# w111liang222/lidar-slam-detection

Hardware: AMD Instinct MI355X
Metric: registered points/sec (120k-pt scan vs 1e7-pt map, full iterate-to-converge) (higher is better)
Workload: dtype f32 per-point geometry / f64 transforms and reductions

## Files before the change

### lidar-slam-detection_amd/csrc/batch.hip

```cpp
#include <sched.h>
#include <stdlib.h>

#include <chrono>
#include <deque>
#include <vector>

#include "eskf.h"
#include "lio_common.h"

using namespace lio;

int engine_resume_update(lio_engine* e, const double* x_now26, const double* x_prop26, const double* P_prop, int i, int converge, int t);
void engine_count_passes(lio_engine* e, int* n_pass, int* n_knn);
int engine_joint_register_device(lio_engine* e, const void* d_raw, uint32_t n_raw, double lidar_beg_time, double state26[26], double cov[529]);
struct lio_comm;
extern "C" int lio_comm_world(const lio_comm*);
extern "C" {
int engine_seq_prepare(lio_engine* e, uint32_t n_raw, double lidar_beg_time, int* ekf_inited);
void engine_seq_params(lio_engine* e, double* laser_cov, int* maximum_iter, int* degenerate_detect_en, float* leaf_surf, float* leaf_map, int* static_map,
                       double* travel, double last_pos_lid[3]);
int engine_seq_finish(lio_engine* e, const double x26[26], const double P529[529], int n_ds, int n_pass, int n_knn, int n_eff, int degenerate, int inserted,
                      uint32_t n_add, uint32_t map_err, uint32_t bound);
int engine_seq_resume(lio_engine* e, const double* x_now26, const double* x_prop26, const double* P_prop, int i, int converge, int t);
int engine_seq_has_lru(lio_engine* e);
int engine_fastlio_front(lio_engine* e, const void** d_raw, uint32_t* n_raw, double* beg, double state26[26], double cov529[529]);
void engine_fastlio_back(lio_engine* e);
}

namespace {

struct Group {
    hipStream_t stream = nullptr;
    std::vector<lio_engine*> eng;
    std::vector<lio_engine*> sub_eng;
    double* d_local32 = nullptr;
    double* d_gathered = nullptr;
    char* d_ds_send = nullptr;
    char* d_ds_all = nullptr;
    int ds_world = 0;
    MapRef* d_rowmaps = nullptr;
    std::vector<MapRef> rowmap_rows;
    char* d_block = nullptr;
    char* h_block = nullptr;
    size_t block_bytes = 0;
    SlotDesc* d_desc = nullptr;
    SlotDesc* h_desc = nullptr;
    EskfDev* d_ctrl = nullptr;
    EskfDev* h_ctrl = nullptr;
    hipGraphExec_t exec[5] = {nullptr, nullptr, nullptr, nullptr, nullptr};
    const void* graph_table = nullptr;
    int graph_stencil = 0;
    lio_batch_result* h_res = nullptr;
    lio_batch_result* h_res_dev = nullptr;
    std::vector<int> job_of_slot;
    float4* d_rawbuf = nullptr;
    MapRef* d_maps = nullptr;
    MapRef* h_maps = nullptr;
    SeqDev* d_seq = nullptr;
    SeqDev* h_seq = nullptr;
    std::vector<int> seq_path;
    int any_lru = 0;
    int n_active = 0;
    int launched_passes = 4;
    uint32_t seq = 0;
    uint32_t max_n_raw = 0;
    BatchTimer* bt = nullptr;
};

}

struct lio_batch {
    lio_map* map = nullptr;
    int device = 0;
    int n_slots = 0;
    uint32_t max_raw = 0, max_ds = 0;
    int pred_passes = 4;
    bool broken = false;
    int use_graph = 1;
    int count_touched = 0;
    std::vector<lio_map*> maps;
    lio_comm* comm = nullptr;
    int world = 1;
    int rank = 0;
    int split_ds = 1;
    uint32_t ds_cap = 0;
    uint32_t ds_seen_max = 0;
    bool ds_cap_full = false;
    uint64_t n_ds_cut = 0;
    int (*gather_hook)(void*, const double*, double*, uint32_t, void*) = nullptr;
    void* gather_ctx = nullptr;
    bool joint = false;
    bool sequences = false;
    std::vector<lio_scan_job> fl_jobs;
    std::vector<double> fl_state, fl_cov;
    std::vector<Group> groups;
    double t_submit = 0, t_wait = 0, t_collect = 0;
    uint64_t n_rounds = 0;
};

static void fill_mapref(MapRef& r, const lio_map* m);

namespace {

const MapRef* joint_rowmaps(lio_batch* b, Group& g) {
    const int M = (int)b->maps.size(), B = b->n_slots;
    if (M < 2) return nullptr;
    for (int m = 1; m < M; m++)
        if (b->maps[m]->stencil_id != b->maps[0]->stencil_id || b->maps[m]->stencil.n != b->maps[0]->stencil.n) return nullptr;
    std::vector<MapRef> now((size_t)M);
    for (int m = 0; m < M; m++) {
        memset(&now[m], 0, sizeof(MapRef));
        fill_mapref(now[m], b->maps[m]);
    }
    bool fresh = g.d_rowmaps != nullptr && (int)g.rowmap_rows.size() == M;
    for (int m = 0; m < M && fresh; m++) fresh = memcmp(&g.rowmap_rows[m], &now[m], sizeof(MapRef)) == 0;
    if (fresh) return g.d_rowmaps;
    std::vector<MapRef> rows((size_t)M * B);
    for (int m = 0; m < M; m++)
        for (int s = 0; s < B; s++) rows[(size_t)m * B + s] = now[m];
    if (!g.d_rowmaps && hipMalloc(reinterpret_cast<void**>(&g.d_rowmaps), sizeof(MapRef) * rows.size()) != hipSuccess) { g.d_rowmaps = nullptr; return nullptr; }
    if (hipMemcpyAsync(g.d_rowmaps, rows.data(), sizeof(MapRef) * rows.size(), hipMemcpyHostToDevice, g.stream) != hipSuccess) return nullptr;
    if (hipStreamSynchronize(g.stream) != hipSuccess) return nullptr;
    g.rowmap_rows = now;
    return g.d_rowmaps;
}

void fill_desc(SlotDesc& d, lio_scan* sc, EskfDev* d_ctrl, lio_batch_result* d_res) {
    d.max_ds = sc->max_ds;
    d.partial_blocks = sc->partial_blocks;
    d.sd = sc->dev;
    d.keys_a = sc->keys_a; d.keys_b = sc->keys_b; d.vals_a = sc->vals_a; d.vals_b = sc->vals_b;
    d.hist = sc->hist; d.blockcnt = sc->blockcnt; d.hpos = sc->hpos; d.longlist = sc->longlist; d.tie_list = sc->tie_list;
    d.sorted = sc->sorted; d.ds_body = sc->ds_body; d.ds_world = sc->ds_world; d.nn_pts = sc->nn_pts; d.normvec = sc->normvec;
    d.nn_cnt = sc->nn_cnt; d.selected = sc->selected; d.partial = sc->partial;
    d.host_nds = sc->host_nds_dev;
    d.ctrl = d_ctrl;
    d.result = d_res;
}

void fill_ctrl(EskfDev& c, const double* x26, const double* P529, double R, int max_iter, int degenerate_detect_en, int joint = 0) {
    c.joint = joint;
    memcpy(c.x, x26, sizeof(double) * 26);
    memcpy(c.P, P529, sizeof(double) * 529);
    for (int k = 0; k < kEkN; k++) c.limit[k] = 0.001;
    c.R = R;
    c.maximum_iter = max_iter;
    c.degenerate_detect_en = degenerate_detect_en;
    c.is_degenerate = 0;
    ek_begin(c);
}

void group_free(Group& g) {
    for (lio_engine* e : g.eng) lio_engine_destroy(e);
    for (lio_engine* e : g.sub_eng) lio_engine_destroy(e);
    if (g.d_local32) hipFree(g.d_local32);
    if (g.d_gathered) hipFree(g.d_gathered);
    if (g.d_ds_send) hipFree(g.d_ds_send);
    if (g.d_ds_all) hipFree(g.d_ds_all);
    if (g.d_rowmaps) hipFree(g.d_rowmaps);
    for (int k = 0; k < 5; k++)
        if (g.exec[k]) hipGraphExecDestroy(g.exec[k]);
    if (g.d_block) hipFree(g.d_block);
    if (g.d_rawbuf) hipFree(g.d_rawbuf);
    if (g.h_block) hipHostFree(g.h_block);
    if (g.d_seq) hipFree(g.d_seq);
    if (g.h_seq) hipHostFree(g.h_seq);
    if (g.h_res) hipHostFree(g.h_res);
    if (g.stream) hipStreamDestroy(g.stream);
    if (g.bt) {
        if (g.bt->created)
            for (int c = 0; c < BatchTimer::kClasses; c++)
                for (int i = 0; i < BatchTimer::kPool; i++) { hipEventDestroy(g.bt->ev[c][i][0]); hipEventDestroy(g.bt->ev[c][i][1]); }
        delete g.bt;
    }
}

const float4* stage_host_raw(lio_batch* b, Group& g, int slot, const lio_scan_job& job, int* rc) {
    *rc = LIO_OK;
    if (!g.d_rawbuf) {
        if (hipMalloc(reinterpret_cast<void**>(&g.d_rawbuf), sizeof(float4) * (size_t)b->max_raw * (size_t)b->n_slots) != hipSuccess) {
            set_error("lio_batch: no memory for the raw ring of LIO_JOB_HOST_RAW jobs (%d x %u points)", b->n_slots, b->max_raw);
            *rc = LIO_E_DEVICE;
            return nullptr;
        }
    }
    float4* dst = g.d_rawbuf + (size_t)slot * b->max_raw;
    if (hipMemcpyAsync(dst, job.d_raw, sizeof(float4) * (size_t)job.n_raw, hipMemcpyHostToDevice, g.stream) != hipSuccess) {
        set_error("lio_batch: copy of a LIO_JOB_HOST_RAW cloud failed: %s", hipGetErrorString(hipGetLastError()));
        *rc = LIO_E_DEVICE;
        return nullptr;
    }
    return dst;
}

int submit(lio_batch* b, Group& g, lio_scan_job* jobs, int first, int n, int passes) {
    const int B = b->n_slots;
    g.seq++;
    g.n_active = 0;
    g.max_n_raw = 0;
    g.launched_passes = passes;
    for (int s = 0; s < B; s++) {
        SlotDesc& d = g.h_desc[s];
        d.active = 0;
        g.job_of_slot[s] = -1;
        if (s >= n) continue;
        lio_scan_job& job = jobs[first + s];
        g.job_of_slot[s] = first + s;
        job.rc = LIO_E_INVALID;
        job.n_ds = job.n_pass = job.n_knn_pass = 0;
        if (job.flags & ~LIO_JOB_FLAGS_KNOWN) { set_error("lio_scan_job.flags = 0x%x: unknown bits (a job array that was not zero-initialised?)", job.flags); continue; }
        if (job.flags & LIO_JOB_IDLE) { job.rc = 0; g.job_of_slot[s] = -1; continue; }
        if (!job.state_in || !job.cov_in || (!job.d_raw && job.n_raw)) continue;
        if (job.n_raw > b->max_raw) { set_error("scan of %u points exceeds max_raw %u", job.n_raw, b->max_raw); job.rc = LIO_E_CAPACITY; continue; }
        if (job.n_raw == 0) { job.rc = 2; continue; }
        d.raw = static_cast<const float4*>(job.d_raw);
        if (job.flags & LIO_JOB_HOST_RAW) {
            int src = LIO_OK;
            d.raw = stage_host_raw(b, g, s, job, &src);
            if (src != LIO_OK) { job.rc = src; continue; }
        }
        d.n_raw = job.n_raw;
        d.nblocks = (job.n_raw + 2047u) / 2048u;
        d.active = 1;
        d.seq = g.seq;
        d.min_ds = 5;
        d.reset_cache = (job.flags & LIO_JOB_KEEP_CACHE) ? 0u : 1u;
        fill_ctrl(g.h_ctrl[s], job.state_in, job.cov_in, 0.001 , 4, 1, b->joint ? 1 : 0);
        g.h_res[s].seq = g.seq - 1;
        g.n_active++;
        if (job.n_raw > g.max_n_raw) g.max_n_raw = job.n_raw;
    }
    const int M = (int)b->maps.size();
    for (int m = 1; m < M; m++)
        for (int s = 0; s < B; s++) {
            SlotDesc& d = g.h_desc[(size_t)m * B + s];
            const SlotDesc& p = g.h_desc[s];
            d.raw = p.raw; d.n_raw = p.n_raw; d.nblocks = p.nblocks; d.active = p.active; d.seq = p.seq; d.min_ds = p.min_ds; d.reset_cache = p.reset_cache;
        }
    if (g.n_active == 0) return LIO_OK;
    const bool timed = g.bt && g.bt->on;
    const MapRef* rowmaps = b->joint ? joint_rowmaps(b, g) : nullptr;
    auto enqueue = [&](BatchTimer* bt) -> int {
        LIO_HIP_TRY(hipMemcpyAsync(g.d_block, g.h_block, g.block_bytes, hipMemcpyHostToDevice, g.stream));
        const uint32_t ds_bound = b->max_raw < b->max_ds ? b->max_raw : b->max_ds;
        int rc = LIO_OK;
        if (b->joint && b->world > 1 && b->split_ds) {
            const int per = (B + b->world - 1) / b->world;
            const int s0 = std::min(B, b->rank * per), s1 = std::min(B, s0 + per);
            if (g.ds_world != b->world) {
                if (g.d_ds_send) hipFree(g.d_ds_send);
                if (g.d_ds_all) hipFree(g.d_ds_all);
                g.d_ds_send = g.d_ds_all = nullptr;
                g.ds_world = 0;
                const size_t chunk = (size_t)per * ds_exchange_slot_bytes(ds_bound);
                LIO_HIP_TRY(hipMalloc(reinterpret_cast<void**>(&g.d_ds_send), chunk));
                LIO_HIP_TRY(hipMalloc(reinterpret_cast<void**>(&g.d_ds_all), chunk * (size_t)b->world));
                g.ds_world = b->world;
            }
            if (bt) bt->begin(0);
            if (s1 > s0) rc = vg_downsample_batch(g.stream, g.d_desc + s0, s1 - s0, b->max_raw, b->max_ds, 0.5f, passes);
            if (bt) bt->end(0);
            if (rc != LIO_OK) return rc;
            if (b->ds_cap == 0) {
                const char* k = getenv("LIO_JOINT_DS_CAP");
                const uint32_t want = k ? (uint32_t)strtoul(k, nullptr, 10) : ((ds_bound / 4u + 1023u) & ~1023u);
                b->ds_cap = std::min(ds_bound, std::max(k ? 1u : 4096u, want));
            }
            const uint32_t cap = b->ds_cap_full ? ds_bound : b->ds_cap;
            rc = p2plane_batch_exchange_ds(b->comm, b->world, b->gather_hook, b->gather_ctx, g.stream, g.d_desc, B, per, s0, s1, cap, g.d_ds_send, g.d_ds_all);
            if (rc == LIO_OK && s0 > 0) rc = scan_begin_rows(g.stream, g.d_desc, s0);
            if (rc == LIO_OK && s1 < B) rc = scan_begin_rows(g.stream, g.d_desc + s1, B - s1);
            if (rc != LIO_OK) return rc;
        } else {
            if (bt) bt->begin(0);
            rc = vg_downsample_batch(g.stream, g.d_desc, B, b->max_raw, b->max_ds, 0.5f, passes);
            if (bt) bt->end(0);
            if (rc != LIO_OK) return rc;
        }
        if (b->joint) {
            rc = p2plane_batch_share(g.stream, g.d_desc, B, M, ds_bound);
            if (rc == LIO_OK) rc = scan_begin_rows(g.stream, g.d_desc + B, B * (M - 1));
            if (rc != LIO_OK) return rc;
            return p2plane_batch_update_joint(b->maps.data(), M, b->comm, b->world, b->gather_hook, b->gather_ctx, g.stream, g.d_desc, B, ds_bound, 5, g.d_local32, g.d_gathered, bt,
                                              rowmaps);
        }
        return p2plane_batch_update(b->map, g.stream, g.d_desc, B, ds_bound, 5, bt, bt ? b->count_touched : 0);
    };
    if (!b->use_graph || timed || b->joint) return enqueue(timed ? g.bt : nullptr);
    if (g.graph_table != b->map->table || g.graph_stencil != b->map->stencil.n) {
        for (int k = 0; k < 5; k++)
            if (g.exec[k]) { hipGraphExecDestroy(g.exec[k]); g.exec[k] = nullptr; }
        g.graph_table = b->map->table;
        g.graph_stencil = b->map->stencil.n;
    }
    if (!g.exec[passes]) {
        hipGraph_t graph = nullptr;
        LIO_HIP_TRY(hipStreamBeginCapture(g.stream, hipStreamCaptureModeThreadLocal));
        const int rc = enqueue(nullptr);
        const hipError_t e2 = hipStreamEndCapture(g.stream, &graph);
        if (rc != LIO_OK) { if (graph) hipGraphDestroy(graph); return rc; }
        LIO_HIP_TRY(e2);
        LIO_HIP_TRY(hipGraphInstantiate(&g.exec[passes], graph, nullptr, nullptr, 0));
        hipGraphDestroy(graph);
    }
    LIO_HIP_TRY(hipGraphLaunch(g.exec[passes], g.stream));
    return LIO_OK;
}

int wait_group(Group& g, int B) {
    for (int s = 0; s < B; s++) {
        if (!g.h_desc[s].active) continue;
        volatile uint32_t* seq = &g.h_res[s].seq;
        for (uint64_t spin = 0; *seq != g.seq; spin++) {
            __builtin_ia32_pause();
            if (spin > 2000 && (spin & 31) == 0) sched_yield();
            if (spin > 40000000ull) {
                LIO_HIP_TRY(hipStreamSynchronize(g.stream));
                if (*seq != g.seq) { set_error("batch slot %d did not report (seq %u, expected %u)", s, *seq, g.seq); return LIO_E_DEVICE; }
                break;
            }
        }
    }
    __atomic_thread_fence(__ATOMIC_ACQUIRE);
    return LIO_OK;
}

}


extern "C" {

static lio_batch* batch_create_impl(lio_map** maps, int n_maps, lio_comm* comm, int n_slots, int n_groups, uint32_t max_raw, uint32_t max_ds) {
    lio_map* map = n_maps > 0 && maps ? maps[0] : nullptr;
    if (!map || n_maps > 64 || n_slots < 1 || n_slots > 256 || n_groups < 1 || n_groups > 8 || max_raw == 0 || max_ds == 0) { set_error("lio_batch_create: bad argument"); return nullptr; }
    for (int m = 1; m < n_maps; m++)
        if (!maps[m] || maps[m]->device != map->device) { set_error("lio_batch_create_joint: the sub-maps of a batch live on one device"); return nullptr; }
    if (hipSetDevice(map->device) != hipSuccess) { set_error("lio_batch_create: no HIP device %d", map->device); return nullptr; }
    lio_batch* b = new lio_batch();
    b->map = map;
    b->device = map->device;
    b->n_slots = n_slots;
    b->max_raw = max_raw;
    b->max_ds = max_ds;
    b->maps.assign(maps, maps + n_maps);
    b->comm = comm;
    b->world = comm ? lio_comm_world(comm) : 1;
    b->rank = comm ? lio_comm_rank(comm) : 0;
    { const char* k = getenv("LIO_JOINT_SPLIT_DS"); b->split_ds = (k && k[0] == '0') ? 0 : 1; }
    b->joint = n_maps > 1 || comm != nullptr;
    b->groups.resize(n_groups);
    { const char* k = getenv("LIO_BATCH_GRAPH"); b->use_graph = (k && k[0] == '0') ? 0 : 1; }
    bool ok = true;
    const int M = n_maps;
    for (Group& g : b->groups) ok = ok && hipStreamCreateWithFlags(&g.stream, hipStreamNonBlocking) == hipSuccess;
    for (Group& g : b->groups) {
        g.job_of_slot.assign(n_slots, -1);
        const size_t desc_bytes = sizeof(SlotDesc) * (size_t)n_slots * (size_t)M;
        g.block_bytes = desc_bytes + sizeof(EskfDev) * (size_t)n_slots;
        ok = ok && hipMalloc(reinterpret_cast<void**>(&g.d_block), g.block_bytes) == hipSuccess;
        ok = ok && hipHostMalloc(reinterpret_cast<void**>(&g.h_block), g.block_bytes, hipHostMallocDefault) == hipSuccess;
        if (ok) {
            g.d_desc = reinterpret_cast<SlotDesc*>(g.d_block);
            g.h_desc = reinterpret_cast<SlotDesc*>(g.h_block);
            g.d_ctrl = reinterpret_cast<EskfDev*>(g.d_block + desc_bytes);
            g.h_ctrl = reinterpret_cast<EskfDev*>(g.h_block + desc_bytes);
        }
        ok = ok && hipHostMalloc(reinterpret_cast<void**>(&g.h_res), sizeof(lio_batch_result) * n_slots, hipHostMallocMapped) == hipSuccess;
        ok = ok && hipHostGetDevicePointer(reinterpret_cast<void**>(&g.h_res_dev), g.h_res, 0) == hipSuccess;
        if (b->joint) {
            ok = ok && hipMalloc(reinterpret_cast<void**>(&g.d_local32), sizeof(double) * 32 * n_slots) == hipSuccess;
            ok = ok && hipMalloc(reinterpret_cast<void**>(&g.d_gathered), sizeof(double) * 32 * n_slots * (size_t)b->world) == hipSuccess;
        }
        if (!ok) break;
        memset(g.h_block, 0, g.block_bytes);
        memset(g.h_res, 0, sizeof(lio_batch_result) * n_slots);
        ok = hipMemset(g.d_block, 0, g.block_bytes) == hipSuccess;
        for (int s = 0; s < n_slots && ok; s++) {
            lio_engine* e = lio_engine_create_shared(map, max_raw, max_ds);
            if (!e) { ok = false; break; }
            lio_engine_set_flags(e, 1, 0, 0.0, -10.0);
            g.eng.push_back(e);
            fill_desc(g.h_desc[s], lio_engine_scan(e), &g.d_ctrl[s], &g.h_res_dev[s]);
        }
        for (int m = 1; m < M && ok; m++)
            for (int s = 0; s < n_slots && ok; s++) {
                lio_engine* e = lio_engine_create_shared(maps[m], max_raw, max_ds);
                if (!e) { ok = false; break; }
                lio_engine_set_flags(e, 1, 0, 0.0, -10.0);
                g.sub_eng.push_back(e);
                fill_desc(g.h_desc[(size_t)m * n_slots + s], lio_engine_scan(e), &g.d_ctrl[s], nullptr);
            }
        for (int s = 0; s < n_slots && ok && b->joint; s++) {
            std::vector<lio_engine*> others;
            for (int m = 1; m < M; m++) others.push_back(g.sub_eng[(size_t)(m - 1) * n_slots + s]);
            ok = lio_engine_set_joint(g.eng[s], others.empty() ? nullptr : others.data(), (int)others.size(), comm) == LIO_OK;
        }
    }
    if (!ok) {
        set_error("lio_batch_create: device setup failed: %s", hipGetErrorString(hipGetLastError()));
        lio_batch_destroy(b);
        return nullptr;
    }
    {
        const char* q = getenv("GPU_MAX_HW_QUEUES");
        if (n_groups > 1 && (!q || atoi(q) < 8))
            set_warning("lio_batch_create: GPU_MAX_HW_QUEUES=%s -- with fewer than 8 hardware queues the %d rounds in flight mostly serialise (~20 %% slower); "
                        "export GPU_MAX_HW_QUEUES=8 before the process's first HIP call", q ? q : "(unset: 4)", n_groups);
    }
    return b;
}

lio_batch* lio_batch_create(lio_map* map, int n_slots, int n_groups, uint32_t max_raw, uint32_t max_ds) {
    return batch_create_impl(&map, map ? 1 : 0, nullptr, n_slots, n_groups, max_raw, max_ds);
}

lio_batch* lio_batch_create_joint(lio_map** sub_maps, int n_sub_maps, lio_comm* comm, int n_slots, int n_groups, uint32_t max_raw, uint32_t max_ds) {
    return batch_create_impl(sub_maps, n_sub_maps, comm, n_slots, n_groups, max_raw, max_ds);
}

int lio_batch_set_gather_hook(lio_batch* b, lio_gather_fn fn, void* ctx, int rank, int world) {
    if (!b || !fn || world < 1 || rank < 0 || rank >= world) return LIO_E_INVALID;
    if (!b->joint || b->comm) { set_error("lio_batch_set_gather_hook: for a batch made by lio_batch_create_joint without a communicator"); return LIO_E_STATE; }
    hipSetDevice(b->map->device);
    for (auto& g : b->groups) {
        LIO_HIP_TRY(hipStreamSynchronize(g.stream));
        if (g.d_gathered) hipFree(g.d_gathered);
        g.d_gathered = nullptr;
        LIO_HIP_TRY(hipMalloc(reinterpret_cast<void**>(&g.d_gathered), sizeof(double) * 32 * b->n_slots * (size_t)world));
    }
    b->gather_hook = fn;
    b->gather_ctx = ctx;
    b->world = world;
    b->rank = rank;
    return LIO_OK;
}

int lio_batch_exchange_stats(lio_batch* b, uint32_t* chunk_points, uint64_t* jobs_rerun, uint64_t* bytes_per_rank_and_round) {
    if (!b) return LIO_E_INVALID;
    const bool on = b->joint && b->world > 1 && b->split_ds;
    if (chunk_points) *chunk_points = on ? b->ds_cap : 0u;
    if (jobs_rerun) *jobs_rerun = b->n_ds_cut;
    if (bytes_per_rank_and_round) {
        const int per = (b->n_slots + b->world - 1) / b->world;
        *bytes_per_rank_and_round = on && b->ds_cap ? (uint64_t)per * ds_exchange_slot_bytes(b->ds_cap) : 0u;
    }
    return LIO_OK;
}

void lio_batch_destroy(lio_batch* b) {
    if (!b) return;
    hipSetDevice(b->device);
    if (getenv("LIO_BATCH_PROFILE") && b->n_rounds)
        fprintf(stderr, "lio_batch: %llu rounds of %d slots; host per round: submit %.1f us, wait %.1f us, collect %.1f us\n", (unsigned long long)b->n_rounds,
                b->n_slots, 1e6 * b->t_submit / b->n_rounds, 1e6 * b->t_wait / b->n_rounds, 1e6 * b->t_collect / b->n_rounds);
    for (Group& g : b->groups) {
        if (g.stream) hipStreamSynchronize(g.stream);
        group_free(g);
    }
    delete b;
}

int lio_batch_enable_kernel_timing(lio_batch* b, int on) {
    if (!b) return LIO_E_INVALID;
    hipSetDevice(b->device);
    for (Group& g : b->groups) {
        if (!g.bt) { g.bt = new BatchTimer(); g.bt->stream = g.stream; }
        if (on && !g.bt->created) {
            for (int c = 0; c < BatchTimer::kClasses; c++)
                for (int i = 0; i < BatchTimer::kPool; i++) {
                    LIO_HIP_TRY(hipEventCreate(&g.bt->ev[c][i][0]));
                    LIO_HIP_TRY(hipEventCreate(&g.bt->ev[c][i][1]));
                }
            g.bt->created = true;
        }
        g.bt->on = on != 0;
    }
    b->count_touched = (on & 2) ? 1 : 0;
    if (b->count_touched && b->map) { const int rc = map_enable_touch_bits(b->map); if (rc != LIO_OK) return rc; }
    return LIO_OK;
}

int lio_batch_kernel_times(lio_batch* b, lio_batch_times* out, int reset) {
    if (!b || !out) return LIO_E_INVALID;
    memset(out, 0, sizeof(*out));
    for (Group& g : b->groups) {
        if (!g.bt) continue;
        out->downsample_us += g.bt->us[0]; out->knn_us += g.bt->us[1]; out->linearize_us += g.bt->us[2]; out->step_us += g.bt->us[3];
        out->downsample_launches += g.bt->launches[0]; out->knn_launches += g.bt->launches[1]; out->linearize_launches += g.bt->launches[2];
        out->step_launches += g.bt->launches[3];
        out->insert_us += g.bt->us[4];
        out->insert_launches += g.bt->launches[4];
        if (reset)
            for (int c = 0; c < BatchTimer::kClasses; c++) { g.bt->us[c] = 0; g.bt->launches[c] = 0; }
    }
    return LIO_OK;
}

lio_engine* lio_batch_engine(lio_batch* b, int group, int slot) {
    if (!b || group < 0 || group >= (int)b->groups.size() || slot < 0 || slot >= b->n_slots) return nullptr;
    return b->groups[group].eng[slot];
}

int lio_batch_process(lio_batch* b, lio_scan_job* jobs, int n_jobs) {
    if (!b || (!jobs && n_jobs) || n_jobs < 0) return LIO_E_INVALID;
    if (b->sequences) { set_error("lio_batch_process: a sequence batch is driven by lio_batch_sequences_step"); return LIO_E_STATE; }
    hipSetDevice(b->device);
    const int B = b->n_slots;
    int next = 0, first_err = 0;
    std::deque<int> inflight;
    std::vector<int> retry;
    auto note = [&](int rc) { if (rc < 0 && !first_err) first_err = rc; };
    auto collect = [&](Group& g) {
        int need_max = 1;
        for (int s = 0; s < B; s++) {
            const int j = g.job_of_slot[s];
            if (j < 0) continue;
            if (!g.h_desc[s].active) { note(jobs[j].rc); continue; }
            lio_scan_job& job = jobs[j];
            const lio_batch_result& r = g.h_res[s];
            if (r.radix_passes > need_max) need_max = r.radix_passes;
            if (r.radix_passes > g.launched_passes) { retry.push_back(j); continue; }
            lio_engine* e = g.eng[s];
            lio_scan* sc = lio_engine_scan(e);
            sc->have_ds = r.n_ds;
            sc->n_raw = g.h_desc[s].n_raw;
            job.n_ds = r.n_ds;
            job.n_pass = r.n_pass;
            job.n_knn_pass = r.n_knn_pass;
            if (r.err & 4) {
                hipMemsetAsync(&sc->dev->err, 0, 4, g.stream);
                b->n_ds_cut++;
                retry.push_back(j);
                continue;
            }
            if (r.err & 1) {
                set_error("downsampled scan exceeds max_ds %u", b->max_ds);
                hipMemsetAsync(&sc->dev->err, 0, 4, g.stream);
                job.rc = LIO_E_CAPACITY;
                note(job.rc);
                continue;
            }
            if ((uint32_t)r.n_ds > b->ds_seen_max) b->ds_seen_max = (uint32_t)r.n_ds;
            if (r.status == EK_SKIPPED) { job.rc = 2; continue; }
            if (r.status == EK_NEEDS_HOST && b->joint && b->gather_hook) {
                set_error("lio_batch (gather hook mode): a scan needs the host-driven joint path, which only exists over a lio_comm");
                job.rc = LIO_E_STATE;
                note(job.rc);
                continue;
            }
            if (r.status == EK_NEEDS_HOST && b->joint) {
                if (!(job.flags & LIO_JOB_KEEP_CACHE)) {
                    scan_forget_cache(sc);
                    for (int m = 1; m < (int)b->maps.size(); m++) scan_forget_cache(lio_engine_scan(g.sub_eng[(size_t)(m - 1) * B + s]));
                }
                double st26[26], cov[529];
                memcpy(st26, job.state_in, sizeof(st26));
                memcpy(cov, job.cov_in, sizeof(cov));
                const void* d_cloud = (job.flags & LIO_JOB_HOST_RAW) ? static_cast<const void*>(g.d_rawbuf + (size_t)s * b->max_raw) : job.d_raw;
                const int rc = engine_joint_register_device(e, d_cloud, job.n_raw, job.lidar_beg_time, st26, cov);
                if (rc < 0) { job.rc = rc; note(rc); continue; }
                engine_count_passes(e, &job.n_pass, &job.n_knn_pass);
                if (job.state_out) memcpy(job.state_out, st26, sizeof(st26));
                job.rc = rc;
                continue;
            }
            if (r.status == EK_NEEDS_HOST) {
                const int rc = engine_resume_update(e, r.state, job.state_in, job.cov_in, r.loop_i, r.loop_converge, r.loop_t);
                if (rc != LIO_OK) { job.rc = rc; note(rc); continue; }
                int np = 0, nk = 0;
                engine_count_passes(e, &np, &nk);
                job.n_pass += np;
                job.n_knn_pass += nk;
                if (job.state_out) lio_engine_get_state(e, job.state_out);
                job.rc = 3;
                continue;
            }
            if (job.state_out) memcpy(job.state_out, r.state, sizeof(double) * 26);
            job.rc = 3;
        }
        if (need_max > 4) need_max = 4;
        b->pred_passes = need_max;
        if (b->joint && b->world > 1 && b->split_ds && b->ds_seen_max && !getenv("LIO_JOINT_DS_CAP")) {
            const uint32_t ds_bound = b->max_raw < b->max_ds ? b->max_raw : b->max_ds;
            const uint32_t want = (b->ds_seen_max + b->ds_seen_max / 4u + 1023u) & ~1023u;
            b->ds_cap = std::min(ds_bound, std::max(4096u, want));
        }
    };
    using clk = std::chrono::steady_clock;
    auto secs = [](clk::time_point a, clk::time_point c) { return std::chrono::duration<double>(c - a).count(); };
    auto bail = [&](int rc) {
        for (auto& gg : b->groups) hipStreamSynchronize(gg.stream);
        inflight.clear();
        return rc;
    };
    for (size_t gi = 0; gi < b->groups.size() && next < n_jobs; gi++) {
        const int n = n_jobs - next < B ? n_jobs - next : B;
        const auto t0 = clk::now();
        const int rc = submit(b, b->groups[gi], jobs, next, n, b->pred_passes);
        b->t_submit += secs(t0, clk::now());
        b->n_rounds++;
        if (rc != LIO_OK) return bail(rc);
        next += n;
        inflight.push_back((int)gi);
    }
    while (!inflight.empty()) {
        const int gi = inflight.front();
        inflight.pop_front();
        Group& g = b->groups[gi];
        const auto t0 = clk::now();
        if (g.n_active) {
            const int rc = wait_group(g, B);
            if (rc != LIO_OK) return bail(rc);
        }
        if (g.bt && g.bt->on) { hipStreamSynchronize(g.stream); g.bt->resolve(); }
        const auto t1 = clk::now();
        collect(g);
        const auto t2 = clk::now();
        b->t_wait += secs(t0, t1);
        b->t_collect += secs(t1, t2);
        if (next < n_jobs) {
            const int n = n_jobs - next < B ? n_jobs - next : B;
            const int rc = submit(b, g, jobs, next, n, b->pred_passes);
            b->t_submit += secs(t2, clk::now());
            b->n_rounds++;
            if (rc != LIO_OK) return bail(rc);
            next += n;
            inflight.push_back(gi);
        }
    }
    const std::vector<int> todo = retry;
    retry.clear();
    b->ds_cap_full = true;
    for (const int j : todo) {
        Group& g = b->groups[0];
        int rc = submit(b, g, jobs, j, 1, 4);
        if (rc == LIO_OK && g.n_active) rc = wait_group(g, B);
        if (rc != LIO_OK) { b->ds_cap_full = false; return bail(rc); }
        collect(g);
    }
    b->ds_cap_full = false;
    for (const int j : retry) { jobs[j].rc = LIO_E_DEVICE; note(LIO_E_DEVICE); }
    return first_err;
}

static void fill_mapref(MapRef& r, const lio_map* m) {
    r.table = m->table; r.cap = m->cap; r.pending = m->pending; r.created = m->created; r.pool = m->pool; r.pool_seq = m->pool_seq; r.tie_mode = m->tie_mode; r.md = m->dev;
    r.slot_of_point = m->slot_of_point; r.stage = m->stage; r.pool_cap = m->pool_cap;
    r.touch = m->touch; r.prev_touch = m->prev_touch; r.lru_log = m->lru_log; r.log_mask = m->lru_log_cap ? m->lru_log_cap - 1 : 0;
    r.free_items = m->free_items; r.free_in = m->free_in; r.free_cap = m->free_cap;
    r.first_touch = m->first_touch; r.lru_g = m->lru_g; r.lru_rec = m->lru_rec;
    r.lru_capacity = (uint32_t)m->lru_capacity; r.lru_max_distance = m->lru_max_distance;
    r.mask = m->table_mask; r.inv_res = m->inv_res; r.res = m->res; r.key_mode = m->key_mode; r.max_voxels = (uint32_t)m->max_voxels;
    r.stencil_id = m->stencil_id;
}

lio_batch* lio_batch_create_sequences(int device, float resolution, int stencil, uint64_t max_points, uint64_t max_voxels, int n_slots, int n_groups,
                                      uint32_t max_raw, uint32_t max_ds) {
    if (n_slots < 1 || n_slots > 256 || n_groups < 1 || n_groups > 8 || max_raw == 0 || max_ds == 0 || max_points == 0 || max_voxels == 0) {
        set_error("lio_batch_create_sequences: bad argument");
        return nullptr;
    }
    const uint32_t ds_bound = max_raw < max_ds ? max_raw : max_ds;
    if (ds_bound > max_points || ds_bound > (1u << 20)) { set_error("lio_batch_create_sequences: a scan's %u downsampled points exceed the maps' insert scratch", ds_bound); return nullptr; }
    if (hipSetDevice(device) != hipSuccess) { set_error("lio_batch_create_sequences: no HIP device %d", device); return nullptr; }
    lio_batch* b = new lio_batch();
    b->device = device;
    b->n_slots = n_slots;
    b->max_raw = max_raw;
    b->max_ds = max_ds;
    b->sequences = true;
    { const char* k = getenv("LIO_BATCH_GRAPH"); b->use_graph = (k && k[0] == '0') ? 0 : 1; }
    b->groups.resize(n_groups);
    bool ok = true;
    for (Group& g : b->groups) ok = ok && hipStreamCreateWithFlags(&g.stream, hipStreamNonBlocking) == hipSuccess;
    for (Group& g : b->groups) {
        g.job_of_slot.assign(n_slots, -1);
        g.seq_path.assign(n_slots, 0);
        const size_t desc_bytes = sizeof(SlotDesc) * (size_t)n_slots, ctrl_bytes = sizeof(EskfDev) * (size_t)n_slots;
        g.block_bytes = desc_bytes + ctrl_bytes + sizeof(MapRef) * (size_t)n_slots;
        ok = ok && hipMalloc(reinterpret_cast<void**>(&g.d_block), g.block_bytes) == hipSuccess;
        ok = ok && hipHostMalloc(reinterpret_cast<void**>(&g.h_block), g.block_bytes, hipHostMallocDefault) == hipSuccess;
        ok = ok && hipMalloc(reinterpret_cast<void**>(&g.d_seq), sizeof(SeqDev) * (size_t)n_slots) == hipSuccess;
        ok = ok && hipHostMalloc(reinterpret_cast<void**>(&g.h_seq), sizeof(SeqDev) * (size_t)n_slots, hipHostMallocDefault) == hipSuccess;
        ok = ok && hipHostMalloc(reinterpret_cast<void**>(&g.h_res), sizeof(lio_batch_result) * n_slots, hipHostMallocMapped) == hipSuccess;
        ok = ok && hipHostGetDevicePointer(reinterpret_cast<void**>(&g.h_res_dev), g.h_res, 0) == hipSuccess;
        if (!ok) break;
        g.d_desc = reinterpret_cast<SlotDesc*>(g.d_block);
        g.h_desc = reinterpret_cast<SlotDesc*>(g.h_block);
        g.d_ctrl = reinterpret_cast<EskfDev*>(g.d_block + desc_bytes);
        g.h_ctrl = reinterpret_cast<EskfDev*>(g.h_block + desc_bytes);
        g.d_maps = reinterpret_cast<MapRef*>(g.d_block + desc_bytes + ctrl_bytes);
        g.h_maps = reinterpret_cast<MapRef*>(g.h_block + desc_bytes + ctrl_bytes);
        memset(g.h_block, 0, g.block_bytes);
        memset(g.h_res, 0, sizeof(lio_batch_result) * n_slots);
        memset(g.h_seq, 0, sizeof(SeqDev) * (size_t)n_slots);
        ok = hipMemset(g.d_block, 0, g.block_bytes) == hipSuccess && hipMemset(g.d_seq, 0, sizeof(SeqDev) * (size_t)n_slots) == hipSuccess;
        for (int s = 0; s < n_slots && ok; s++) {
            lio_engine* e = lio_engine_create(device, resolution, stencil, max_points, max_voxels, max_raw, max_ds);
            if (!e) { ok = false; break; }
            lio_engine_set_device_loop(e, 1);
            g.eng.push_back(e);
            fill_desc(g.h_desc[s], lio_engine_scan(e), &g.d_ctrl[s], &g.h_res_dev[s]);
        }
    }
    if (!ok) {
        set_error("lio_batch_create_sequences: device setup failed: %s", hipGetErrorString(hipGetLastError()));
        lio_batch_destroy(b);
        return nullptr;
    }
    b->map = lio_engine_map(b->groups[0].eng[0]);
    return b;
}

int lio_batch_sequences_step(lio_batch* b, lio_scan_job* jobs, int n_jobs, double* cov_out) {
    if (!b || !jobs) return LIO_E_INVALID;
    if (!b->sequences) { set_error("lio_batch_sequences_step: for a batch made by lio_batch_create_sequences"); return LIO_E_STATE; }
    if (b->broken) { set_error("lio_batch_sequences_step: an earlier step failed after part of it had run on the device; the sessions' maps hold that sweep, their engines do not -- destroy the batch"); return LIO_E_STATE; }
    const int B = b->n_slots, G = (int)b->groups.size();
    if (n_jobs != B * G) { set_error("lio_batch_sequences_step: %d jobs for %d sessions (job j is the next scan of session j; LIO_JOB_IDLE marks a session without one)", n_jobs, B * G); return LIO_E_INVALID; }
    hipSetDevice(b->device);
    int first_err = 0;
    auto note = [&](int rc) { if (rc < 0 && !first_err) first_err = rc; };
    const uint32_t ds_bound = b->max_raw < b->max_ds ? b->max_raw : b->max_ds;
    const int passes = b->pred_passes;
    for (int gi = 0; gi < G; gi++) {
        Group& g = b->groups[gi];
        g.seq++;
        g.n_active = 0;
        g.max_n_raw = 0;
        g.launched_passes = passes;
        g.any_lru = 0;
        StencilArgs stencils[4];
        int stencil_ids[4], n_st = 0;
        for (int s = 0; s < B; s++) {
            SlotDesc& d = g.h_desc[s];
            d.active = 0;
            g.job_of_slot[s] = gi * B + s;
            g.seq_path[s] = -1000;
            lio_scan_job& job = jobs[gi * B + s];
            job.n_ds = job.n_pass = job.n_knn_pass = 0;
            job.rc = LIO_E_INVALID;
            if (job.flags & ~LIO_JOB_FLAGS_KNOWN) { set_error("lio_scan_job.flags = 0x%x: unknown bits (a job array that was not zero-initialised?)", job.flags); note(job.rc); continue; }
            if (job.flags & LIO_JOB_IDLE) { job.rc = 0; g.job_of_slot[s] = -1; continue; }
            if (!job.state_in || !job.cov_in || (!job.d_raw && job.n_raw)) { note(job.rc); continue; }
            if (job.flags & LIO_JOB_HOST_RAW) { set_error("lio_batch_sequences_step: LIO_JOB_HOST_RAW is a static-batch flag (a session's sweeps arrive through lio_fastlio_pcl_stage / _commit)"); note(job.rc); continue; }
            if (job.n_raw > b->max_raw) { set_error("scan of %u points exceeds max_raw %u", job.n_raw, b->max_raw); job.rc = LIO_E_CAPACITY; note(job.rc); continue; }
            lio_engine* e = g.eng[s];
            int ekf_inited = 0;
            const int path = engine_seq_prepare(e, job.n_raw, job.lidar_beg_time, &ekf_inited);
            g.seq_path[s] = path;
            if (path < 0) { job.rc = path; note(path); continue; }
            if (path == 0 || path == 2) { job.rc = path; if (job.state_out) memcpy(job.state_out, job.state_in, sizeof(double) * 26); if (cov_out) memcpy(cov_out + (size_t)(gi * B + s) * 529, job.cov_in, sizeof(double) * 529); continue; }
            if (path == 10) {
                lio_engine_set_state(e, job.state_in);
                lio_engine_set_cov(e, job.cov_in);
                const int rc = lio_engine_process_scan_device(e, job.d_raw, job.n_raw, job.lidar_beg_time);
                job.rc = rc;
                note(rc);
                if (rc >= 0) {
                    lio_timings tm;
                    lio_engine_timings(e, &tm);
                    job.n_ds = tm.n_ds; job.n_pass = tm.n_pass; job.n_knn_pass = tm.n_knn_pass;
                    if (job.state_out) lio_engine_get_state(e, job.state_out);
                    if (cov_out) lio_engine_get_cov(e, cov_out + (size_t)(gi * B + s) * 529);
                }
                continue;
            }
            lio_map* m = lio_engine_map(e);
            double laser_cov = 0.001, travel = 0, last_pos_lid[3];
            int maximum_iter = 4, deg_en = 1, static_map = 0;
            float leaf_surf = 0.5f, leaf_map = 0.5f;
            engine_seq_params(e, &laser_cov, &maximum_iter, &deg_en, &leaf_surf, &leaf_map, &static_map, &travel, last_pos_lid);
            if (leaf_surf != 0.5f || maximum_iter != 4) { set_error("sequence batch: the round is built for filter_size_surf 0.5 and NUM_MAX_ITERATIONS 4"); job.rc = LIO_E_STATE; note(job.rc); g.seq_path[s] = LIO_E_STATE; continue; }
            if (m->lru_capacity && m->tomb_bound > m->table_cap / 4) {
                const int rc = map_rebuild(m, g.stream);
                if (rc != LIO_OK) { job.rc = rc; note(rc); g.seq_path[s] = rc; continue; }
            }
            d.raw = static_cast<const float4*>(job.d_raw);
            d.n_raw = job.n_raw;
            d.nblocks = (job.n_raw + 2047u) / 2048u;
            d.active = 1;
            d.seq = g.seq;
            d.min_ds = 5;
            d.reset_cache = 0;
            fill_ctrl(g.h_ctrl[s], job.state_in, job.cov_in, laser_cov, maximum_iter, deg_en, 0);
            MapRef& r = g.h_maps[s];
            fill_mapref(r, m);
            r.stamp_base = (unsigned long long)(m->n_batches + 1) << kStampIdxBits;
            r.do_insert = static_map ? 0u : 1u;
            r.ekf_inited = (uint32_t)ekf_inited;
            r.map_leaf = leaf_map;
            r.travel_prev = travel;
            for (int i = 0; i < 3; i++) r.last_pos_lid[i] = last_pos_lid[i];
            if (m->lru_capacity) g.any_lru = 1;
            int k = 0;
            while (k < n_st && stencil_ids[k] != m->stencil_id) k++;
            if (k == n_st && n_st < 4) { stencils[n_st] = m->stencil; stencil_ids[n_st] = m->stencil_id; n_st++; }
            else if (k == n_st) { set_error("sequence batch: more than four different stencils in one round"); job.rc = LIO_E_STATE; note(job.rc); d.active = 0; g.seq_path[s] = LIO_E_STATE; continue; }
            g.h_res[s].seq = g.seq - 1;
            g.n_active++;
            if (job.n_raw > g.max_n_raw) g.max_n_raw = job.n_raw;
        }
        if (g.n_active == 0) continue;
        const bool timed = g.bt && g.bt->on;
        auto enqueue = [&](BatchTimer* bt) -> int {
            LIO_HIP_TRY(hipMemcpyAsync(g.d_block, g.h_block, g.block_bytes, hipMemcpyHostToDevice, g.stream));
            if (bt) bt->begin(0);
            int rc = vg_downsample_batch(g.stream, g.d_desc, B, b->max_raw, b->max_ds, 0.5f, passes);
            if (bt) bt->end(0);
            if (rc == LIO_OK) rc = p2plane_seq_update(g.stream, g.d_maps, g.d_desc, B, ds_bound, 5, stencils, stencil_ids, n_st, bt);
            if (bt) bt->begin(4);
            if (rc == LIO_OK) rc = p2plane_seq_insert(g.stream, g.d_maps, g.d_desc, g.d_seq, B, ds_bound, g.any_lru);
            if (bt) bt->end(4);
            if (rc != LIO_OK) return rc;
            LIO_HIP_TRY(hipMemcpyAsync(g.h_seq, g.d_seq, sizeof(SeqDev) * (size_t)B, hipMemcpyDeviceToHost, g.stream));
            return LIO_OK;
        };
        int rc = LIO_OK;
        if (!b->use_graph || timed) {
            rc = enqueue(timed ? g.bt : nullptr);
        } else {
            int sig = g.any_lru ? 1 : 0;
            for (int k = 0; k < n_st; k++) sig = sig * 131 + stencil_ids[k] + 1;
            if (g.graph_stencil != sig) {
                for (int k = 0; k < 5; k++)
                    if (g.exec[k]) { hipGraphExecDestroy(g.exec[k]); g.exec[k] = nullptr; }
                g.graph_stencil = sig;
            }
            if (!g.exec[passes]) {
                hipGraph_t graph = nullptr;
                rc = hipStreamBeginCapture(g.stream, hipStreamCaptureModeThreadLocal) == hipSuccess ? LIO_OK : LIO_E_DEVICE;
                if (rc == LIO_OK) {
                    rc = enqueue(nullptr);
                    const hipError_t e2 = hipStreamEndCapture(g.stream, &graph);
                    if (rc == LIO_OK && e2 != hipSuccess) rc = LIO_E_DEVICE;
                    if (rc == LIO_OK && hipGraphInstantiate(&g.exec[passes], graph, nullptr, nullptr, 0) != hipSuccess) rc = LIO_E_DEVICE;
                    if (graph) hipGraphDestroy(graph);
                }
                if (rc == LIO_E_DEVICE) set_error("sequence batch: capturing the round failed: %s", hipGetErrorString(hipGetLastError()));
            }
            if (rc == LIO_OK && hipGraphLaunch(g.exec[passes], g.stream) != hipSuccess) { set_error("sequence batch: hipGraphLaunch: %s", hipGetErrorString(hipGetLastError())); rc = LIO_E_DEVICE; }
        }
        if (rc != LIO_OK) {
            for (int k = 0; k <= gi; k++) (void)hipStreamSynchronize(b->groups[k].stream);
            for (int k = 0; k < G; k++)
                for (int s2 = 0; s2 < B; s2++) {
                    lio_scan_job& j2 = jobs[k * B + s2];
                    const bool in_round = k <= gi && b->groups[k].seq_path[s2] == 11;
                    if (k > gi || in_round) j2.rc = (j2.flags & LIO_JOB_IDLE) && !(j2.flags & ~LIO_JOB_FLAGS_KNOWN) ? 0 : LIO_E_DEVICE;
                }
            if (gi > 0) b->broken = true;
            return rc;
        }
        b->n_rounds++;
    }
    int need_max = 1;
    for (int gi = 0; gi < G; gi++) {
        Group& g = b->groups[gi];
        if (g.n_active == 0) continue;
        LIO_HIP_TRY(hipStreamSynchronize(g.stream));
        if (g.bt && g.bt->on) g.bt->resolve();
        for (int s = 0; s < B; s++) {
            if (!g.h_desc[s].active) continue;
            lio_scan_job& job = jobs[gi * B + s];
            const lio_batch_result& r = g.h_res[s];
            const SeqDev& q = g.h_seq[s];
            lio_engine* e = g.eng[s];
            lio_scan* sc = lio_engine_scan(e);
            double* cov_dst = cov_out ? cov_out + (size_t)(gi * B + s) * 529 : nullptr;
            if (r.seq != g.seq) { set_error("sequence batch: slot %d did not report", s); job.rc = LIO_E_DEVICE; note(job.rc); continue; }
            if (r.radix_passes > need_max) need_max = r.radix_passes;
            if (r.radix_passes > g.launched_passes) {
                lio_engine_set_state(e, job.state_in);
                lio_engine_set_cov(e, job.cov_in);
                const int rc = lio_engine_process_scan_device(e, job.d_raw, job.n_raw, job.lidar_beg_time);
                job.rc = rc;
                note(rc);
                if (rc >= 0) {
                    lio_timings tm;
                    lio_engine_timings(e, &tm);
                    job.n_ds = tm.n_ds; job.n_pass = tm.n_pass; job.n_knn_pass = tm.n_knn_pass;
                    if (job.state_out) lio_engine_get_state(e, job.state_out);
                    if (cov_dst) lio_engine_get_cov(e, cov_dst);
                }
                continue;
            }
            sc->have_ds = r.n_ds;
            sc->n_raw = g.h_desc[s].n_raw;
            job.n_ds = r.n_ds;
            job.n_pass = r.n_pass;
            job.n_knn_pass = r.n_knn_pass;
            if (r.err & 1) {
                set_error("downsampled scan exceeds max_ds %u", b->max_ds);
                hipMemsetAsync(&sc->dev->err, 0, 4, g.stream);
                job.rc = LIO_E_CAPACITY;
                note(job.rc);
                continue;
            }
            if (r.status == EK_SKIPPED) {
                job.rc = 2;
                if (job.state_out) memcpy(job.state_out, job.state_in, sizeof(double) * 26);
                if (cov_dst) memcpy(cov_dst, job.cov_in, sizeof(double) * 529);
                continue;
            }
            if (r.status == EK_NEEDS_HOST) {
                const int rc = engine_seq_resume(e, r.state, job.state_in, job.cov_in, r.loop_i, r.loop_converge, r.loop_t);
                if (rc < 0) { job.rc = rc; note(rc); continue; }
                int np = 0, nk = 0;
                engine_count_passes(e, &np, &nk);
                job.n_pass += np;
                job.n_knn_pass += nk;
                if (job.state_out) lio_engine_get_state(e, job.state_out);
                if (cov_dst) lio_engine_get_cov(e, cov_dst);
                job.rc = rc;
                continue;
            }
            const int rc = engine_seq_finish(e, r.state, q.P, r.n_ds, r.n_pass, r.n_knn_pass, r.n_eff, r.degenerate, (int)q.go, q.n_add, q.go ? q.map_err : 0u, (uint32_t)r.n_ds );
            if (job.state_out) memcpy(job.state_out, r.state, sizeof(double) * 26);
            if (cov_dst) memcpy(cov_dst, q.P, sizeof(double) * 529);
            job.rc = rc;
            note(rc);
        }
    }
    if (need_max > 4) need_max = 4;
    b->pred_passes = need_max;
    return first_err;
}

}

int lio_batch_fastlio_main(lio_batch* b, int* rc_out) {
    if (!b || !rc_out) return LIO_E_INVALID;
    if (!b->sequences) { set_error("lio_batch_fastlio_main: for a batch made by lio_batch_create_sequences"); return LIO_E_STATE; }
    const int B = b->n_slots, G = (int)b->groups.size(), n = B * G;
    hipSetDevice(b->device);
    b->fl_jobs.assign((size_t)n, lio_scan_job{});
    b->fl_state.resize((size_t)n * 26);
    b->fl_cov.resize((size_t)n * 529);
    int first_err = 0, n_ready = 0;
    std::vector<char> ready((size_t)n, 0);
    for (int j = 0; j < n; j++) {
        lio_engine* e = b->groups[j / B].eng[j % B];
        lio_scan_job& job = b->fl_jobs[j];
        job.flags = LIO_JOB_IDLE;
        const void* d_raw = nullptr;
        uint32_t n_raw = 0;
        double beg = 0;
        const int fr = engine_fastlio_front(e, &d_raw, &n_raw, &beg, &b->fl_state[(size_t)j * 26], &b->fl_cov[(size_t)j * 529]);
        rc_out[j] = fr;
        if (fr < 0 && !first_err) first_err = fr;
        if (fr != 1000) continue;
        job.flags = 0;
        job.d_raw = d_raw;
        job.n_raw = n_raw;
        job.lidar_beg_time = beg;
        job.state_in = &b->fl_state[(size_t)j * 26];
        job.cov_in = &b->fl_cov[(size_t)j * 529];
        job.state_out = nullptr;
        ready[j] = 1;
        n_ready++;
    }
    if (n_ready) {
        const int rc = lio_batch_sequences_step(b, b->fl_jobs.data(), n, nullptr);
        if (rc < 0 && !first_err) first_err = rc;
        for (int j = 0; j < n; j++) {
            if (!ready[j]) continue;
            rc_out[j] = b->fl_jobs[j].rc;
            engine_fastlio_back(b->groups[j / B].eng[j % B]);
        }
    }
    return first_err;
}

struct lio_devloop {
    char* d_block = nullptr;
    char* h_block = nullptr;
    size_t block_bytes = 0;
    SlotDesc* d_desc = nullptr;
    SlotDesc* h_desc = nullptr;
    EskfDev* d_ctrl = nullptr;
    EskfDev* h_ctrl = nullptr;
    EskfDev* h_back = nullptr;
    lio_batch_result* h_res = nullptr;
    lio_batch_result* h_res_dev = nullptr;
    static constexpr int kBuckets = 8;
    hipGraphExec_t exec[kBuckets] = {nullptr, nullptr, nullptr, nullptr, nullptr, nullptr, nullptr, nullptr};
    uint32_t seq = 0;
    int stencil_n = 0;
    const void* table = nullptr;
};

void devloop_destroy(lio_devloop* d) {
    if (!d) return;
    for (int k = 0; k < lio_devloop::kBuckets; k++)
        if (d->exec[k]) hipGraphExecDestroy(d->exec[k]);
    if (d->d_block) hipFree(d->d_block);
    if (d->h_block) hipHostFree(d->h_block);
    if (d->h_back) hipHostFree(d->h_back);
    if (d->h_res) hipHostFree(d->h_res);
    delete d;
}

lio_devloop* devloop_create(lio_scan* sc) {
    lio_devloop* d = new lio_devloop();
    d->block_bytes = sizeof(SlotDesc) + sizeof(EskfDev);
    bool ok = hipMalloc(reinterpret_cast<void**>(&d->d_block), d->block_bytes) == hipSuccess &&
              hipHostMalloc(reinterpret_cast<void**>(&d->h_block), d->block_bytes, hipHostMallocDefault) == hipSuccess &&
              hipHostMalloc(reinterpret_cast<void**>(&d->h_back), sizeof(EskfDev), hipHostMallocDefault) == hipSuccess &&
              hipHostMalloc(reinterpret_cast<void**>(&d->h_res), sizeof(lio_batch_result), hipHostMallocMapped) == hipSuccess &&
              hipHostGetDevicePointer(reinterpret_cast<void**>(&d->h_res_dev), d->h_res, 0) == hipSuccess;
    if (!ok) { devloop_destroy(d); return nullptr; }
    d->d_desc = reinterpret_cast<SlotDesc*>(d->d_block);
    d->h_desc = reinterpret_cast<SlotDesc*>(d->h_block);
    d->d_ctrl = reinterpret_cast<EskfDev*>(d->d_block + sizeof(SlotDesc));
    d->h_ctrl = reinterpret_cast<EskfDev*>(d->h_block + sizeof(SlotDesc));
    memset(d->h_block, 0, d->block_bytes);
    memset(d->h_res, 0, sizeof(lio_batch_result));
    fill_desc(*d->h_desc, sc, d->d_ctrl, d->h_res_dev);
    return d;
}

int devloop_update(lio_devloop* d, lio_map* m, lio_scan* sc, const double* x26, const double* P529, double R, int max_iter, int degenerate_detect_en,
                   const EskfDev** out) {
    SlotDesc& desc = *d->h_desc;
    desc.active = 1;
    desc.min_ds = 0;
    desc.reset_cache = 0;
    desc.n_raw = sc->n_raw;
    desc.nblocks = 0;
    desc.seq = ++d->seq;
    fill_ctrl(*d->h_ctrl, x26, P529, R, max_iter, degenerate_detect_en);
    const uint32_t bound = sc->have_ds > 0 ? (uint32_t)sc->have_ds : (sc->n_raw && sc->n_raw < sc->max_ds ? sc->n_raw : sc->max_ds);
    hipStream_t st = sc->stream;
    auto enqueue = [&](uint32_t ds_bound) -> int {
        LIO_HIP_TRY(hipMemcpyAsync(d->d_block, d->h_block, d->block_bytes, hipMemcpyHostToDevice, st));
        const int rc = p2plane_batch_update(m, st, d->d_desc, 1, ds_bound, max_iter + 1, nullptr, 0);
        if (rc != LIO_OK) return rc;
        LIO_HIP_TRY(hipMemcpyAsync(d->h_back, d->d_ctrl, sizeof(EskfDev), hipMemcpyDeviceToHost, st));
        return LIO_OK;
    };
    static const bool use_graph = []() { const char* k = getenv("LIO_BATCH_GRAPH"); return !(k && k[0] == '0'); }();
    if (use_graph && max_iter == 4) {
        if (d->stencil_n != m->stencil.n || d->table != m->table) {
            for (int k = 0; k < lio_devloop::kBuckets; k++)
                if (d->exec[k]) { hipGraphExecDestroy(d->exec[k]); d->exec[k] = nullptr; }
            d->stencil_n = m->stencil.n;
            d->table = m->table;
        }
        int bk = 0;
        while (bk < lio_devloop::kBuckets - 1 && (2048u << bk) < bound) bk++;
        uint32_t cap_b = 2048u << bk;
        if (cap_b > sc->max_ds || bk == lio_devloop::kBuckets - 1) cap_b = sc->max_ds;
        if (cap_b < bound) cap_b = bound;
        if (!d->exec[bk]) {
            hipGraph_t graph = nullptr;
            LIO_HIP_TRY(hipStreamBeginCapture(st, hipStreamCaptureModeThreadLocal));
            const int rc = enqueue(cap_b);
            const hipError_t e2 = hipStreamEndCapture(st, &graph);
            if (rc != LIO_OK) { if (graph) hipGraphDestroy(graph); return rc; }
            LIO_HIP_TRY(e2);
            LIO_HIP_TRY(hipGraphInstantiate(&d->exec[bk], graph, nullptr, nullptr, 0));
            hipGraphDestroy(graph);
        }
        LIO_HIP_TRY(hipGraphLaunch(d->exec[bk], st));
    } else {
        const int rc = enqueue(bound);
        if (rc != LIO_OK) return rc;
    }
    LIO_HIP_TRY(hipStreamSynchronize(st));
    *out = d->h_back;
    return LIO_OK;
}
```

Before: 6.126 billion.

## Balance small batch calls across stream groups and upload only live slot descriptors

Adds a batch planner. When a call has fewer than two full rounds of jobs per group, it splits them evenly into rounds that are a multiple of the group count, so every stream gets work instead of leaving some groups idle. In balanced mode the predicted pass count is held at the call-wide maximum. For non-joint batches, the host-to-device copy of descriptors and control blocks covers only the live slots and is issued once, outside the enqueue lambda. Smaller rounds may use less of each launch's parallelism, and the graph replay path may now skip the copy that used to run inside it.

Result: slower. 4.437 billion (-27.6%).

```diff
diff --git a/lidar-slam-detection_amd/csrc/batch.hip b/lidar-slam-detection_amd/csrc/batch.hip
--- a/lidar-slam-detection_amd/csrc/batch.hip
+++ b/lidar-slam-detection_amd/csrc/batch.hip
@@ -5,6 +5,7 @@
 #include <deque>
 #include <vector>
 
+#include "batch_plan.h"
 #include "eskf.h"
 #include "lio_common.h"
 
@@ -77,6 +78,7 @@
     int pred_passes = 4;
     bool broken = false;
     int use_graph = 1;
+    BatchPlanMode plan_mode;
     int count_touched = 0;
     std::vector<lio_map*> maps;
     lio_comm* comm = nullptr;
@@ -95,7 +97,7 @@
     std::vector<double> fl_state, fl_cov;
     std::vector<Group> groups;
     double t_submit = 0, t_wait = 0, t_collect = 0;
-    uint64_t n_rounds = 0;
+    uint64_t n_rounds = 0, n_round_jobs = 0;
 };
 
 static void fill_mapref(MapRef& r, const lio_map* m);
@@ -240,8 +242,12 @@
     if (g.n_active == 0) return LIO_OK;
     const bool timed = g.bt && g.bt->on;
     const MapRef* rowmaps = b->joint ? joint_rowmaps(b, g) : nullptr;
+    if (!b->joint) {
+        const size_t live_bytes = (size_t)(reinterpret_cast<char*>(g.h_ctrl) - g.h_block) + sizeof(EskfDev) * (size_t)(n < B ? n : B);
+        LIO_HIP_TRY(hipMemcpyAsync(g.d_block, g.h_block, live_bytes, hipMemcpyHostToDevice, g.stream));
+    }
     auto enqueue = [&](BatchTimer* bt) -> int {
-        LIO_HIP_TRY(hipMemcpyAsync(g.d_block, g.h_block, g.block_bytes, hipMemcpyHostToDevice, g.stream));
+        if (b->joint) LIO_HIP_TRY(hipMemcpyAsync(g.d_block, g.h_block, g.block_bytes, hipMemcpyHostToDevice, g.stream));
         const uint32_t ds_bound = b->max_raw < b->max_ds ? b->max_raw : b->max_ds;
         int rc = LIO_OK;
         if (b->joint && b->world > 1 && b->split_ds) {
@@ -350,6 +356,7 @@
     b->joint = n_maps > 1 || comm != nullptr;
     b->groups.resize(n_groups);
     { const char* k = getenv("LIO_BATCH_GRAPH"); b->use_graph = (k && k[0] == '0') ? 0 : 1; }
+    b->plan_mode = batch_plan_mode(getenv("LIO_BATCH_PLAN"));
     bool ok = true;
     const int M = n_maps;
     for (Group& g : b->groups) ok = ok && hipStreamCreateWithFlags(&g.stream, hipStreamNonBlocking) == hipSuccess;
@@ -451,8 +458,9 @@
     if (!b) return;
     hipSetDevice(b->device);
     if (getenv("LIO_BATCH_PROFILE") && b->n_rounds)
-        fprintf(stderr, "lio_batch: %llu rounds of %d slots; host per round: submit %.1f us, wait %.1f us, collect %.1f us\n", (unsigned long long)b->n_rounds,
-                b->n_slots, 1e6 * b->t_submit / b->n_rounds, 1e6 * b->t_wait / b->n_rounds, 1e6 * b->t_collect / b->n_rounds);
+        fprintf(stderr, "lio_batch: %llu rounds of %d slots, %.1f jobs per round (slot fill %.2f); host per round: submit %.1f us, wait %.1f us, collect %.1f us\n",
+                (unsigned long long)b->n_rounds, b->n_slots, (double)b->n_round_jobs / b->n_rounds, (double)b->n_round_jobs / ((double)b->n_rounds * b->n_slots),
+                1e6 * b->t_submit / b->n_rounds, 1e6 * b->t_wait / b->n_rounds, 1e6 * b->t_collect / b->n_rounds);
     for (Group& g : b->groups) {
         if (g.stream) hipStreamSynchronize(g.stream);
         group_free(g);
@@ -510,6 +518,8 @@
     std::deque<int> inflight;
     std::vector<int> retry;
     auto note = [&](int rc) { if (rc < 0 && !first_err) first_err = rc; };
+    bool balanced = false;
+    int call_need = 1;
     auto collect = [&](Group& g) {
         int need_max = 1;
         for (int s = 0; s < B; s++) {
@@ -579,7 +589,8 @@
             job.rc = 3;
         }
         if (need_max > 4) need_max = 4;
-        b->pred_passes = need_max;
+        if (need_max > call_need) call_need = need_max;
+        b->pred_passes = balanced ? call_need : need_max;
         if (b->joint && b->world > 1 && b->split_ds && b->ds_seen_max && !getenv("LIO_JOINT_DS_CAP")) {
             const uint32_t ds_bound = b->max_raw < b->max_ds ? b->max_raw : b->max_ds;
             const uint32_t want = (b->ds_seen_max + b->ds_seen_max / 4u + 1023u) & ~1023u;
@@ -593,12 +604,19 @@
         inflight.clear();
         return rc;
     };
-    for (size_t gi = 0; gi < b->groups.size() && next < n_jobs; gi++) {
-        const int n = n_jobs - next < B ? n_jobs - next : B;
+    bool any_keep_cache = false;
+    for (int j = 0; j < n_jobs && !any_keep_cache; j++) any_keep_cache = (jobs[j].flags & LIO_JOB_KEEP_CACHE) != 0;
+    const bool may_replan = batch_may_replan(any_keep_cache, b->joint, b->sequences, b->plan_mode);
+    const std::vector<int> plan = batch_plan(n_jobs, B, (int)b->groups.size(), may_replan, b->plan_mode.min_round);
+    balanced = may_replan && n_jobs < 2 * B * (int)b->groups.size();
+    size_t round = 0;
+    for (size_t gi = 0; gi < b->groups.size() && round < plan.size(); gi++) {
+        const int n = plan[round++];
         const auto t0 = clk::now();
         const int rc = submit(b, b->groups[gi], jobs, next, n, b->pred_passes);
         b->t_submit += secs(t0, clk::now());
         b->n_rounds++;
+        b->n_round_jobs += (uint64_t)n;
         if (rc != LIO_OK) return bail(rc);
         next += n;
         inflight.push_back((int)gi);
@@ -618,11 +636,12 @@
         const auto t2 = clk::now();
         b->t_wait += secs(t0, t1);
         b->t_collect += secs(t1, t2);
-        if (next < n_jobs) {
-            const int n = n_jobs - next < B ? n_jobs - next : B;
+        if (round < plan.size()) {
+            const int n = plan[round++];
             const int rc = submit(b, g, jobs, next, n, b->pred_passes);
             b->t_submit += secs(t2, clk::now());
             b->n_rounds++;
+            b->n_round_jobs += (uint64_t)n;
             if (rc != LIO_OK) return bail(rc);
             next += n;
             inflight.push_back(gi);
diff --git a/lidar-slam-detection_amd/csrc/batch_plan.h b/lidar-slam-detection_amd/csrc/batch_plan.h
--- /dev/null
+++ b/lidar-slam-detection_amd/csrc/batch_plan.h
@@ -0,0 +1,47 @@
+#pragma once
+
+#include <stdlib.h>
+#include <string.h>
+
+#include <vector>
+
+namespace lio {
+
+constexpr int kBatchPlanMinRound = 1;
+
+struct BatchPlanMode {
+    bool fill = false;
+    int min_round = 0;
+};
+inline BatchPlanMode batch_plan_mode(const char* env) {
+    BatchPlanMode m;
+    if (!env) return m;
+    if (strcmp(env, "fill") == 0) m.fill = true;
+    else if (strncmp(env, "min:", 4) == 0 && atoi(env + 4) >= 1) m.min_round = atoi(env + 4);
+    return m;
+}
+
+inline bool batch_may_replan(bool any_keep_cache, bool joint, bool sequences, const BatchPlanMode& mode) {
+    return !any_keep_cache && !joint && !sequences && !mode.fill;
+}
+
+inline std::vector<int> batch_plan(int n_jobs, int n_slots, int n_groups, bool may_replan, int min_round = 0) {
+    std::vector<int> sizes;
+    if (n_jobs <= 0 || n_slots < 1 || n_groups < 1) return sizes;
+    const long long B = n_slots, G = n_groups, n = n_jobs;
+    const long long r_min = (n + B - 1) / B;
+    if (!may_replan || n >= 2 * B * G) {
+        for (long long left = n; left > 0; left -= B) sizes.push_back((int)(left < B ? left : B));
+        return sizes;
+    }
+    const long long m = min_round >= 1 ? min_round : kBatchPlanMinRound;
+    long long R = (r_min + G - 1) / G * G;
+    const long long cap = n / m;
+    if (R > cap) R = cap;
+    if (R < r_min) R = r_min;
+    const long long base = n / R, extra = n % R;
+    for (long long r = 0; r < R; r++) sizes.push_back((int)(base + (r < extra ? 1 : 0)));
+    return sizes;
+}
+
+}
```
